# sabbirhossainujjal/LLMVoX

Hardware: AMD Instinct MI355X
Metric: speech tokens/sec (+ 24kHz audio samples/sec = 320 x tokens/s; p50 first-chunk latency) (higher is better)
Workload: dtype bf16

## Files before the change

llmvox_amd/csrc/ar_kernels.hip:

```cpp
#include "ar_plan.h"

#pragma clang fp contract(off)

namespace lvx {

#ifdef LVX_TIMING
constexpr int TS_BLOCKS = 1024;
__device__ uint64_t g_lvx_ts[16 * 4 * TS_BLOCKS * 4];
#define TS_DECL uint64_t ts_[2] = {0, 0}
#define TS_MARK(i) do { if (threadIdx.x == 0) ts_[i] = __builtin_amdgcn_s_memrealtime(); } while (0)
#define TS_SAVE(tag, layer, blk)                                                                    \
  do {                                                                                               \
    if (threadIdx.x == 0) {                                                                          \
      const uint64_t te_ = __builtin_amdgcn_s_memrealtime();                                         \
      const uint64_t hw_ = (uint64_t)__builtin_amdgcn_s_getreg((31 << 11) | 4) |                    \
                           ((uint64_t)__builtin_amdgcn_s_getreg((3 << 11) | 20) << 32);              \
      uint64_t* p_ = g_lvx_ts + ((size_t)(((tag) * 4 + (layer)) * TS_BLOCKS + min((int)(blk), TS_BLOCKS - 1))) * 4; \
      p_[0] = ts_[0]; p_[1] = ts_[1]; p_[2] = te_; p_[3] = hw_;                                      \
    }                                                                                                \
  } while (0)
#else
#define TS_DECL do {} while (0)
#define TS_MARK(i) do {} while (0)
#define TS_SAVE(tag, layer, blk) do {} while (0)
// ... 907 lines not shown
}
__device__ __forceinline__ void slot_update_bf16(float& m, float& l, f32x2_t (&o)[12], float sc, const uint4 (&vp)[3],
                                                 bool valid) {
  uint32_t v[12];
#pragma unroll
  for (int i = 0; i < 3; ++i) { v[4 * i] = vp[i].x; v[4 * i + 1] = vp[i].y; v[4 * i + 2] = vp[i].z; v[4 * i + 3] = vp[i].w; }
  if (!valid) return;
  const float mn = fmaxf(m, sc);
  const float alpha = __builtin_amdgcn_exp2f((m - mn) * 1.4426950408889634f);
  const float p = __builtin_amdgcn_exp2f((sc - mn) * 1.4426950408889634f);
  l = l * alpha + p;
  const f32x2_t a2 = f32x2_t{alpha, alpha}, p2 = f32x2_t{p, p};
#pragma unroll
  for (int j = 0; j < 12; ++j) {
    const f32x2_t vv = f32x2_t{__uint_as_float(v[j] << 16), __uint_as_float(v[j] & 0xffff0000u)};
    o[j] = __builtin_elementwise_fma(p2, vv, o[j] * a2);
  }
  m = mn;
}
__device__ __forceinline__ void slot_softmax_step_bf16(float& m, float& l, f32x2_t (&o)[12], const QSplit& qs,
                                                       const uint4 (&kp)[3], const uint4 (&vp)[3], bool valid) {
  slot_update_bf16(m, l, o, slot_score_bf16(qs, kp), vp, valid);
}

__device__ __forceinline__ float slot_fold_wave(float m, float& l, float (&o)[24]) {
  const float M = wave_max(m);
  const float f = (m == -INFINITY) ? 0.f : expf(m - M);
  l *= f;
#pragma unroll
  for (int i = 0; i < 24; ++i) o[i] *= f;
  return M;
}

template <typename TKV, int DEPTH, int NW, bool QKV = false>
__global__ __launch_bounds__(NW * 64) void ar_attn_v2_kernel(ArState st, int layer, int ns_max, int direct,
                                                         int selcopy) {
  constexpr int TK = NW * 16;
  constexpr bool SLOT = sizeof(TKV) < 4;
  static_assert(!QKV || (NW == 4 && sizeof(TKV) == 4), "the K-split c_attn: the fp32 parity mode's 4-wave blocks");
  constexpr int QH = QKV ? (3 * HD + NW * 64 - 1) / (NW * 64) : 1;
  __shared__ float wm_s[NW], wl_s[NW];
  __shared__ float wo_s[NW][4][HD];
  __shared__ float qs_s[QKV ? HD : 1];
  __shared__ __attribute__((aligned(16))) TKV kvh_s[QKV ? 2 : 1][QKV ? HD : 1];
  const int sp = blockIdx.x, head = blockIdx.y, b = blockIdx.z;
  const int tid = threadIdx.x, wave = tid >> 6, lane = tid & 63;
  TS_DECL;
  TS_MARK(0);
  const int4 ri = selcopy ? st.rowinfo_n[b] : st.rowinfo[b];
  float pq[QH][QKV ? 4 : 1];
  if constexpr (QKV) {
#pragma unroll
    for (int h = 0; h < QH; ++h) {
      const int e = min(tid + NW * 64 * h, 3 * HD - 1);
      const float* pp = st.qkvp + (size_t)b * (3 * D) + (e / HD) * D + head * HD + e % HD;
#pragma unroll
      for (int k = 0; k < 4; ++k) pq[h][k] = pp[(size_t)k * st.max_streams * (3 * D)];
    }
  }
  const bool cp = selcopy && sp == 0 && head == 0 && tid == 0;
  int jn = 0;
  if (cp) {
    jn = st.rowx_n[b].x;
    st.rowinfo[b] = ri;
    st.selrow[b] = 1u;
    if (b == 0) *st.selp = 0u;
  }
  auto copy_tail = [&]() {
    if (cp) st.rowx[b] = make_int2(jn, plan_tok(st, b, jn + 1));
  };
  const int s = ri.x;
  if (s < 0) {
    copy_tail();
    if (direct == ATTN_F32_ROWS && sp == 0 && tid < HD) st.part_o[(size_t)(b * N_HEAD + head) * NSPLIT * HD + tid] = 0.f;
    return;
  }
  const int t = ri.y + 1;
  const int ns = min(ns_max, (t + ATK - 1) / ATK);
  if (sp >= ns) return;
  const int chunk = SLOT ? (((t + ns - 1) / ns + ATK - 1) / ATK) * ATK : (t + ns - 1) / ns;
  const int k0 = sp * chunk, k1 = min(t, k0 + chunk);
  const size_t base = kv_at(layer, st.kv_chunks, st.max_streams, s, head, 0);
  const size_t cstride = (size_t)st.max_streams * N_HEAD * KV_CHUNK * HD;
  const TKV* __restrict__ Kg = reinterpret_cast<const TKV*>(st.kc) + base;
  const TKV* __restrict__ Vg = reinterpret_cast<const TKV*>(st.vc) + base;
  auto krow = [&](int k) { return (size_t)(k / KV_CHUNK) * cstride + (size_t)(k % KV_CHUNK) * HD; };
  const int part = tid & 3, kq = tid >> 2;
  float q[24];
  if constexpr (!QKV) {
    const float* qg = st.q + (size_t)b * D + head * HD + part * 24;
#pragma unroll
    for (int i = 0; i < 24; i += 4) {
      const float4 v = *reinterpret_cast<const float4*>(qg + i);
      q[i] = v.x * 0.10206207261596575f; q[i + 1] = v.y * 0.10206207261596575f;
      q[i + 2] = v.z * 0.10206207261596575f; q[i + 3] = v.w * 0.10206207261596575f;
    }
  }
  float m = -INFINITY, l = 0.f, o[24];
#pragma unroll
  for (int i = 0; i < 24; ++i) o[i] = 0.f;
  KvPiece<TKV> kpr[DEPTH][3], vpr[DEPTH][3];
  const int klast = ((k1 - 1) / ATK) * ATK;
  auto issue = [&](int kb, KvPiece<TKV>(&kp)[3], KvPiece<TKV>(&vp)[3]) {
    if constexpr (SLOT) {
      const size_t off = (size_t)min((kb / KV_CHUNK) + (kq / KV_CHUNK), klast / KV_CHUNK) * cstride +
                         (size_t)(kq % KV_CHUNK) * HD + part * 24;
#pragma unroll
      for (int i = 0; i < 3; ++i) {
        kp[i].load(Kg + off + i * 8);
        vp[i].load(Vg + off + i * 8);
      }
      return;
    }
    const int key = min(kb + kq, k1 - 1);
#pragma unroll
    for (int i = 0; i < 3; ++i) {
      kp[i].load(Kg + krow(key) + part * 24 + i * 8);
      vp[i].load(Vg + krow(key) + part * 24 + i * 8);
    }
  };
  constexpr bool BF = SLOT && sizeof(TKV) == 2;
  f32x2_t o2[BF ? 12 : 1];
// ... 44 lines not shown
    const float p = valid ? expf(sc - mn) : 0.f;
    l = l * alpha + wave_sum(part == 0 ? p : 0.f);
#pragma unroll
    for (int i = 0; i < 24; ++i) o[i] = fmaf(valid ? p : 0.f, valid ? vf[i] : 0.f, o[i] * alpha);
    m = mn;
  };
#pragma unroll
  for (int d = 0; d < DEPTH; ++d) issue(k0 + d * TK, kpr[d], vpr[d]);
  if constexpr (QKV) {
#pragma unroll
    for (int h = 0; h < QH; ++h) {
      const int e = tid + NW * 64 * h;
      float v = 0.f;
#pragma unroll
      for (int k = 0; k < 4; ++k) v += pq[h][k];
      if (e < HD) {
        qs_s[e] = v;
      } else if (e < 3 * HD && k1 == t) {
        const int which = e / HD - 1, d = e % HD;
        TKV hv;
        if constexpr (sizeof(TKV) == 4) hv = v;
        else if constexpr (sizeof(TKV) == 2) hv = f32_to_bf16(v);
        else hv = f32_to_fp8(v);
        kvh_s[which][d] = hv;
        reinterpret_cast<TKV*>(which ? st.vc : st.kc)[base + krow(ri.y) + d] = hv;
      }
    }
    asm volatile("s_waitcnt lgkmcnt(0)" ::: "memory");
    __builtin_amdgcn_s_barrier();
    asm volatile("" ::: "memory");
#pragma unroll
    for (int i = 0; i < 24; ++i) q[i] = qs_s[part * 24 + i] * 0.10206207261596575f;
  }
  if constexpr (BF) qsplit_make(q, qsp);
  for (int kb = k0; kb < k1; kb += DEPTH * TK) {
#pragma unroll
    for (int d = 0; d < DEPTH; ++d) {
      if (DEPTH == 2 && d > 0 && kb + d * TK >= k1) break;
      tile(kb + d * TK, kpr[d], vpr[d]);
      issue(kb + (d + DEPTH) * TK, kpr[d], vpr[d]);
      if (DEPTH > 2) __builtin_amdgcn_sched_barrier(0);
    }
  }
  if constexpr (BF) {
#pragma unroll
    for (int j = 0; j < 12; ++j) { o[2 * j] = o2[j].x; o[2 * j + 1] = o2[j].y; }
  }
  if constexpr (SLOT) {
    m = slot_fold_wave(m, l, o);
    l = wave_sum(part == 0 ? l : 0.f);
  }
#pragma unroll
  for (int i = 0; i < 24; ++i) {
    float v = o[i];
    v += dpp_f32<0x128>(v);
    v += dpp_f32<0x124>(v);
    o[i] = v;
  }
  if ((lane & 15) < 4) {
#pragma unroll
    for (int i = 0; i < 24; ++i) wo_s[wave][lane >> 4][(lane & 3) * 24 + i] = o[i];
  }
  TS_MARK(1);
  if (lane == 0) { wm_s[wave] = m; wl_s[wave] = l; }
  __syncthreads();
  TS_SAVE(2, layer, sp + gridDim.x * (head + N_HEAD * b));
  copy_tail();
  if (tid < HD) {
    float M = wm_s[0];
#pragma unroll
    for (int w = 1; w < NW; ++w) M = fmaxf(M, wm_s[w]);
    float ov = 0.f, lv = 0.f;
#pragma unroll
    for (int w = 0; w < NW; ++w) {
      const float f = (wm_s[w] == -INFINITY) ? 0.f : expf(wm_s[w] - M);
      ov += f * ((wo_s[w][0][tid] + wo_s[w][1][tid]) + (wo_s[w][2][tid] + wo_s[w][3][tid]));
      lv += f * wl_s[w];
    }
    if (direct == ATTN_F32_ROWS) {
      st.part_o[(size_t)(b * N_HEAD + head) * NSPLIT * HD + tid] = ov * (1.0f / lv);
      return;
    }
    if (direct) {
      st.xn[direct == ATTN_XN_PACKED ? xfrag(b, head * HD + tid, D) : (size_t)b * D + head * HD + tid] = f32_to_bf16(ov * (1.0f / lv));
      return;
    }
    st.part_o[((size_t)(b * N_HEAD + head) * NSPLIT + sp) * HD + tid] = ov;
    if (tid == 0) {
      float* ml = st.part_ml + ((size_t)(b * N_HEAD + head) * NSPLIT + sp) * 2;
      ml[0] = M;
      ml[1] = lv;
    }
  }
}

__device__ __forceinline__ void argmax_row(const ArState& st, int b, int4 ri, float* sv, float* sv2, int* si) {
  const int tid = threadIdx.x, wave = tid >> 6, lane = tid & 63;
  const float4* lg = reinterpret_cast<const float4*>(st.logits + (size_t)b * VOCAB);
  Best bt{-INFINITY, -INFINITY, 0x7fffffff};
#pragma unroll
  for (int j = 0; j < VOCAB / 1024; ++j) {
    const float4 v = lg[j * 256 + tid];
    const int i0 = (j * 256 + tid) * 4;
    bt = best_merge(bt, Best{v.x, -INFINITY, i0});
    bt = best_merge(bt, Best{v.y, -INFINITY, i0 + 1});
    bt = best_merge(bt, Best{v.z, -INFINITY, i0 + 2});
    bt = best_merge(bt, Best{v.w, -INFINITY, i0 + 3});
  }
  bt = best_wave(bt);
  if (lane == 0) { sv[wave] = bt.v; sv2[wave] = bt.v2; si[wave] = bt.i; }
  __syncthreads();
  if (wave == 0) {
    Best r{sv[0], sv2[0], si[0]};
    for (int w = 1; w < 4; ++w) r = best_merge(r, Best{sv[w], sv2[w], si[w]});
    r = softmax_ties(st.logits + (size_t)b * VOCAB, r, lane);
    if (lane == 0) argmax_commit(st, b, ri, r);
  }
}

__global__ __launch_bounds__(256) void ar_argmax_kernel(ArState st) {
  __shared__ float sv[4], sv2[4];
  __shared__ int si[4];
  const int b = blockIdx.x;
  const int4 ri = st.rowinfo[b];
  if (ri.x < 0) return;
  argmax_row(st, b, ri, sv, sv2, si);
// ... 181 lines not shown

__device__ __forceinline__ void embed_row(const GemvArgs& a, int4 ri, int lane, float4 (&v)[3], float* rden = nullptr) {
  if (ri.x < 0) {
#pragma unroll
    for (int j = 0; j < 3; ++j) v[j] = make_float4(0.f, 0.f, 0.f, 0.f);
    return;
  }
  const int p = ri.y, prev = ri.w;
  const int tok = ri.z < 0 ? 384 : ri.z;
  float4 pe[3];
  const float* wr_ = a.wpe + (size_t)p * D;
#pragma unroll
  for (int j = 0; j < 3; ++j) pe[j] = *reinterpret_cast<const float4*>(wr_ + j * 256 + lane * 4);
#pragma unroll
  for (int j = 0; j < 3; ++j) {
    const int k = j * 256 + lane * 4;
    v[j] = j == 0 ? *reinterpret_cast<const float4*>(a.text_table + (size_t)tok * TEXT_DIM + k)
                  : *reinterpret_cast<const float4*>(a.codebook + (size_t)prev * SPEECH_DIM + (k - TEXT_DIM));
  }
  if (ri.z < 0 && lane == 0) atomicOr(a.st.err, 2);
  float ss = 0.f;
#pragma unroll
  for (int j = 0; j < 3; ++j) {
    if (j > 0 && p == 0) v[j] = make_float4(0.f, 0.f, 0.f, 0.f);
    ss += (v[j].x * v[j].x + v[j].y * v[j].y) + (v[j].z * v[j].z + v[j].w * v[j].w);
  }
  const float den = fmaxf(sqrtf(wave_sum(ss)), 1e-8f);
  if (rden) *rden = 1.0f / den;
#pragma unroll
  for (int j = 0; j < 3; ++j)
    v[j] = make_float4(v[j].x / den + pe[j].x, v[j].y / den + pe[j].y, v[j].z / den + pe[j].z, v[j].w / den + pe[j].w);
}


template <int MODE>
__global__ __launch_bounds__(256) LVX_LOADS_FIRST void ar_rows_kernel(GemvArgs a) {
  const int tid = threadIdx.x, wave = tid >> 6, lane = tid & 63;
  const int b = blockIdx.x * (blockDim.x >> 6) + wave;
  if (b >= a.B) return;
  TS_DECL;
  TS_MARK(0);
  float4 g[3], v[3];
#pragma unroll
  for (int j = 0; j < 3; ++j) g[j] = *reinterpret_cast<const float4*>(a.ln_w + j * 256 + lane * 4);
  if (MODE == RMODE_LN || MODE == RMODE_LN_Y || MODE == RMODE_LN_Y_F32) {
    XRow<MODE == RMODE_LN_Y_F32 ? GIN_LN_Y : MODE> r;
    xrow_issue(a, b, lane, r);
    __builtin_amdgcn_sched_barrier(0);
    xrow_sum(r, v);
    if (MODE == RMODE_LN_Y || MODE == RMODE_LN_Y_F32)
#pragma unroll
      for (int j = 0; j < 3; ++j) *reinterpret_cast<float4*>(a.st.x + (size_t)b * D + j * 256 + lane * 4) = v[j];
  } else {
    const int4 ri = a.st.rowinfo[b];
    embed_row(a, ri, lane, v);
#pragma unroll
    for (int j = 0; j < 3; ++j) *reinterpret_cast<float4*>(a.st.x + (size_t)b * D + j * 256 + lane * 4) = v[j];
  }
  TS_MARK(1);
  wave_ln_regs(v, g);
  if constexpr (MODE == RMODE_LN_Y_F32 || MODE == RMODE_EMBED_F32) {
#pragma unroll
    for (int j = 0; j < 3; ++j) *reinterpret_cast<float4*>(a.st.h + (size_t)b * D + j * 256 + lane * 4) = v[j];
    return;
  }
  uint2* dst = reinterpret_cast<uint2*>(a.st.xn + (size_t)b * D);
#pragma unroll
  for (int j = 0; j < 3; ++j) {
    if (a.xpk) *reinterpret_cast<uint2*>(a.st.xn + xfrag(b, j * 256 + lane * 4, D)) = pack4_bf16(v[j]);
    else dst[j * 64 + lane] = pack4_bf16(v[j]);
  }
  TS_SAVE(a.N == VOCAB ? 8 : 0, a.layer, blockIdx.x);
}

template <bool F32OUT = false>
__global__ __launch_bounds__(256) LVX_LOADS_FIRST void ar_embed_select_kernel(GemvArgs a) {
  __shared__ float sv[4], sv2[4];
  __shared__ int si[4];
  const int b = blockIdx.x, tid = threadIdx.x, wave = tid >> 6, lane = tid & 63;
  TS_DECL;
  TS_MARK(0);
  int4 ri = a.st.rowinfo[b];
  const int2 rx = a.st.rowx[b];
  const unsigned pend = a.st.selrow[b];
  float4 g[3];
#pragma unroll
  for (int j = 0; j < 3; ++j) g[j] = *reinterpret_cast<const float4*>(a.ln_w + j * 256 + lane * 4);
  const float4* lg = reinterpret_cast<const float4*>(a.st.logits + (size_t)b * VOCAB);
  float4 lv[VOCAB / 1024];
#pragma unroll
  for (int k = 0; k < VOCAB / 1024; ++k) lv[k] = lg[k * 256 + tid];
  Best bt{-INFINITY, -INFINITY, 0x7fffffff};
#pragma unroll
  for (int k = 0; k < VOCAB / 1024; ++k) {
    const int i0 = (k * 256 + tid) * 4;
    bt = best_merge(bt, Best{lv[k].x, -INFINITY, i0});
    bt = best_merge(bt, Best{lv[k].y, -INFINITY, i0 + 1});
    bt = best_merge(bt, Best{lv[k].z, -INFINITY, i0 + 2});
    bt = best_merge(bt, Best{lv[k].w, -INFINITY, i0 + 3});
  }
  bt = best_wave(bt);
  TS_MARK(1);
  if (lane == 0) { sv[wave] = bt.v; sv2[wave] = bt.v2; si[wave] = bt.i; }
// ... 167 lines not shown
    bt = best_merge(bt, Best{lv[k].x, -INFINITY, i0});
    bt = best_merge(bt, Best{lv[k].y, -INFINITY, i0 + 1});
    bt = best_merge(bt, Best{lv[k].z, -INFINITY, i0 + 2});
    bt = best_merge(bt, Best{lv[k].w, -INFINITY, i0 + 3});
  }
  bt = best_wave(bt);
  if (lane == 0) { sv[wave] = bt.v; sv2[wave] = bt.v2; si[wave] = bt.i; }
  __syncthreads();
  int4 rn = ri;
  if (tk) {
    Best r{sv[0], sv2[0], si[0]};
#pragma unroll
    for (int w = 1; w < 4; ++w) r = best_merge(r, Best{sv[w], sv2[w], si[w]});
    r = softmax_ties(a.st.logits + (size_t)b * VOCAB, r, lane);
    const int sl = ri.x, p = ri.y + 1, j = rx.x;
    rn = make_int4(sl, min(p, a.st.max_pos - 1), rx.y, min(max(r.i, 0), VOCAB - 1));
    if (cx == 0 && tid == 0) {
      if (p >= a.st.max_pos) atomicOr(a.st.err, 1);
      if (j < a.st.plan_stride) {
        a.st.tok_plan[(size_t)b * a.st.plan_stride + j] = r.i;
        if (a.st.margin_plan) a.st.margin_plan[(size_t)b * a.st.plan_stride + j] = r.v - r.v2;
      }
      a.st.prev[sl] = r.i;
      a.st.pos[sl] = p;
      a.st.rowstep[b] = j + 1;
    }
  }
  if (cx == 0 && tid == 0) {
    a.st.rowinfo_n[b] = rn;
    a.st.rowx_n[b] = make_int2(tk ? rx.x + 1 : rx.x, 0);
  }
  const float tc = a.q0_code[(size_t)min(max(rn.w, 0), VOCAB - 1) * (3 * D) + n];
  if (wave == 0) {
    float4 v[3];
    float rden = 0.f;
    embed_row(a, rn, lane, v, &rden);
    if (cx == 0) {
#pragma unroll
      for (int j = 0; j < 3; ++j) *reinterpret_cast<float4*>(a.st.x + (size_t)b * D + j * 256 + lane * 4) = v[j];
    }
    float sm = 0.f;
#pragma unroll
    for (int j = 0; j < 3; ++j) sm += (v[j].x + v[j].y) + (v[j].z + v[j].w);
    const float mean = wave_sum(sm) * (1.0f / D);
    float qs = 0.f;
#pragma unroll
    for (int j = 0; j < 3; ++j) {
      const float4 d = make_float4(v[j].x - mean, v[j].y - mean, v[j].z - mean, v[j].w - mean);
      qs += (d.x * d.x + d.y * d.y) + (d.z * d.z + d.w * d.w);
    }
    const float rstd = 1.0f / sqrtf(wave_sum(qs) * (1.0f / D) + 1e-5f);
    if (lane == 0) sst = make_float4(rden, mean, rstd, 0.f);
  }
  __syncthreads();
  const float4 st = sst;
  const float cz = rn.y == 0 ? 0.f : 1.f;
  const float o = rn.x < 0 ? 0.f : st.z * (((tq + cz * tc) * st.x + tpo) - st.y * gq);
  if (n < D) {
    a.st.q[(size_t)b * D + n] = o;
  } else if (rn.x >= 0) {
    const int c = (n - D) % D, which = (n - D) / D;
    const int head = c / HD, d = c - head * HD;
    store_kv(a, which, kv_at(0, a.st.kv_chunks, a.st.max_streams, rn.x, head, rn.y) + d, o);
  }
  TS_SAVE(7, 0, cx + 9 * b);
}

template <int NS>
__global__ __launch_bounds__(256) void ar_merge_bf16_kernel(ArState st, int ns_max, int xpk) {
  __shared__ float cf[N_HEAD * NSPLIT];
  const int b = blockIdx.x, tid = threadIdx.x;
  const int4 ri = st.rowinfo[b];
  float2 ml = make_float2(-INFINITY, 0.f);
  if (tid < N_HEAD * NSPLIT) ml = reinterpret_cast<const float2*>(st.part_ml)[(size_t)b * N_HEAD * NSPLIT + tid];
  float pv[3][NS];
#pragma unroll
  for (int j = 0; j < 3; ++j) {
    const int e = tid + 256 * j, head = e / HD, d = e - head * HD;
    const float* po = st.part_o + ((size_t)(b * N_HEAD + head) * NSPLIT) * HD + d;
#pragma unroll
    for (int i = 0; i < NS; ++i) pv[j][i] = po[(size_t)i * HD];
  }
  if (tid < N_HEAD * NSPLIT) {
    const int ns = ri.x < 0 ? 0 : min(ns_max, (ri.y + 1 + 63) / 64);
    const bool on = (tid & (NSPLIT - 1)) < ns && ml.x != -INFINITY;
// ... 896 lines not shown
      break;
    case OP_LM_HEAD:
      a.W = w.w_lm; a.Wf = w.f_lm; a.N = VOCAB; a.ln_w = w.lnf;
      if (p.ksplit) {
        hipLaunchKernelGGL((ar_rows_kernel<RMODE_LN_Y_F32>), dim3(B), dim3(64), 0, s, a);
        launch_f32b<768, FIN_LN_ROWS, FOUT_LOGITS>(a, s);
      } else {
        launch_f32b<768, FIN_LN, FOUT_LOGITS>(a, s);
      }
      break;
  }
}

template <typename TW>
static bool launch_op(int op, GemvArgs& a, const ArWeights& w, int l, const ArStepPlan& p, hipStream_t s) {
  if (p.path == PATH_F32B || p.path == PATH_BT) {
    if (p.path == PATH_F32B) launch_op_f32b(op, a, w, l, p, s);
    else launch_op_bt(op, a, w, l, p, s);
    return true;
  }
  const int B = p.B;
  const bool ln = p.path == PATH_MFMA_LN, mf = ln || p.path == PATH_MFMA_ROWS, fm = p.fused_mlp;
  a.xpk = p.xpk;
  a.layer = l;
  a.yacc = mf ? a.st.yacc : nullptr;
  a.yfx = fm ? a.st.yfx : nullptr;
  a.add_y = l > 0;
  switch (op) {
    case OP_QKV:
      a.W = w.w_attn[l]; a.Wf = w.f_attn[l]; a.N = 3 * D; a.ln_w = w.ln1[l];
      if (!(p.sel == SEL_ARGMAX || (mf ? p.sel == SEL_EMBED || p.sel == SEL_Q0_ROWS || (ln && p.sel == SEL_LN_GRAN)
                                       : p.sel == SEL_GRAN)))
        ar_plan_bug(p, "c_attn");
      if (l == 0 && p.sel == SEL_LN_GRAN) {
        launch_mfma_ln<MLOUT_QKV, MLMODE_EMBED_SELECT>(a, s);
      } else if (l == 0 && p.sel == SEL_Q0_ROWS) {
        hipLaunchKernelGGL(ar_q0_rows_kernel, dim3(3 * D / 256, B), dim3(256), 0, s, a);
      } else if (l == 0 && p.sel == SEL_EMBED) {
        hipLaunchKernelGGL(ar_embed_select_kernel<>, dim3(B), dim3(256), 0, s, a);
        launch_mfma2<768, M2OUT_QKV>(a, s);
      } else if (ln) {
        if (l == 0) launch_mfma_ln<MLOUT_QKV, MLMODE_EMBED>(a, s);
        else launch_mfma_ln<MLOUT_QKV, MLMODE_LN_Y>(a, s);
      } else if (mf) {
        if (l == 0) hipLaunchKernelGGL((ar_rows_kernel<RMODE_EMBED>), dim3(B), dim3(64), 0, s, a);
        else hipLaunchKernelGGL((ar_rows_kernel<RMODE_LN_Y>), dim3(B), dim3(64), 0, s, a);
        launch_mfma2<768, M2OUT_QKV>(a, s);
      } else if (l == 0 && p.q0_gran) {
        hipLaunchKernelGGL(ar_q0_gran_kernel, dim3(3 * D / 256), dim3(256), 0, s, a);
      } else if (l == 0 && p.sel == SEL_GRAN) {
        launch_gemv<TW, 768, 1, 2, GIN_EMBED_SELECT, GOUT_QKV>(a, s);
      } else if (l == 0) {
        launch_gemv<TW, 768, 1, 2, GIN_EMBED, GOUT_QKV>(a, s);
      } else if (fm) {
        launch_gemv<TW, 768, 1, 2, GIN_LN_Y, GOUT_QKV>(a, s);
      } else {
        launch_gemv<TW, 768, 1, 2, GIN_LN, GOUT_QKV>(a, s);
      }
      break;
    case OP_ATTN:
      launch_attn(a.st, p.kv_dtype, B, l, s, p.nsplit, p.attn_direct, p.selcopy && l == 0, false, p.attn8);
      break;
    case OP_CPROJ:
      a.W = w.w_aproj[l]; a.Wf = w.f_aproj[l]; a.N = D;
      if (mf) {
        if (!ln) a.add_y = 0;
        if (p.nsplit > 1) launch_merge_bf16(a.st, B, p.nsplit, s, a.xpk);
        a.ln_w = w.ln2[l];
        if (!ln) launch_mfma2<768, M2OUT_RESID_STATS>(a, s, true);
        else launch_mfma2<768, M2OUT_RESID>(a, s);
      } else {
        launch_gemv<TW, 768, 1, 1, GIN_MERGE, GOUT_RESID>(a, s);
      }
      break;
    case OP_FC:
      a.W = w.w_fc[l]; a.Wf = w.f_fc[l]; a.N = DFF; a.ln_w = w.ln2[l];
      if (fm) {
        const bf16_t* wfc = reinterpret_cast<const bf16_t*>(w.w_fc[l]);
        const bf16_t* wpk = reinterpret_cast<const bf16_t*>(w.w_mproj_pk[l]);
        if (B <= 1) hipLaunchKernelGGL((ar_mlp_fused_kernel<1, 16>), dim3(DFF / 16), dim3(256), 0, s, a, wfc, wpk);
        else hipLaunchKernelGGL((ar_mlp_fused_kernel<2, 16>), dim3(DFF / 16), dim3(256), 0, s, a, wfc, wpk);
      } else if (ln) {
        launch_mfma_ln<MLOUT_GELU_BF16, MLMODE_LN>(a, s);
      } else if (mf) {
        a.gsum = w.fc_gsum[l];
        launch_mfma2<768, M2OUT_GELU_BF16, M2X_LN_AFTER>(a, s);
      } else {
        launch_gemv<TW, 768, 1, 2, GIN_LN, GOUT_GELU>(a, s);
      }
      break;
    case OP_MPROJ:
      a.W = w.w_mproj[l]; a.Wf = w.f_mproj[l]; a.N = D;
      if (fm) return false;
// ... 322 lines not shown
```

llmvox_amd/csrc/ar_plan.h:

```cpp
#pragma once
#include <stdio.h>
#include <stdlib.h>

#include "lvx_internal.h"

namespace lvx {

enum { OP_QKV = 0, OP_ATTN = 1, OP_CPROJ = 2, OP_FC = 3, OP_MPROJ = 4, OP_LM_HEAD = 5 };
enum { GIN_LN = 0, GIN_H = 1, GIN_MERGE = 2, GIN_EMBED = 3, GIN_LN_Y = 4, GIN_EMBED_SELECT = 5 };
enum { GOUT_QKV = 0, GOUT_RESID = 1, GOUT_GELU = 2, GOUT_LOGITS = 3, GOUT_SPLITK = 6, GOUT_LOGITS_GRAN = 9 };
enum { RMODE_LN = 0, RMODE_EMBED = 3, RMODE_LN_Y = 4, RMODE_LN_Y_F32 = 5, RMODE_EMBED_F32 = 6 };
enum { M2OUT_QKV = 0, M2OUT_RESID = 1, M2OUT_LOGITS = 3, M2OUT_GELU_BF16 = 5, M2OUT_SPLITK = 6, M2OUT_RESID_STATS = 7 };
enum { M2X_NONE = 0, M2X_LN_AFTER = 1 };
enum { MLOUT_QKV = 0, MLOUT_LOGITS = 3, MLOUT_GELU_BF16 = 5 };
enum { MLMODE_LN = 0, MLMODE_EMBED = 3, MLMODE_LN_Y = 4, MLMODE_EMBED_SELECT = 7 };
enum { BIN_LN = 0, BIN_ROWS = 1, BIN_EMBED = 3 };
enum { BOUT_QKV = 0, BOUT_RESID = 1, BOUT_LOGITS = 3, BOUT_GELU_BF16 = 5 };
enum { FIN_LN = 0, FIN_H = 1, FIN_MERGE = 2, FIN_EMBED = 3, FIN_ATTN_ROWS = 4, FIN_LN_ROWS = 6 };
enum { FOUT_QKV = 0, FOUT_RESID = 1, FOUT_GELU = 2, FOUT_LOGITS = 3, FOUT_SPLITK = 6 };
enum { ATTN_PARTIALS = 0, ATTN_XN = 1, ATTN_XN_PACKED = 2, ATTN_F32_ROWS = 3 };

enum ArPath { PATH_GEMV, PATH_MFMA_LN, PATH_MFMA_ROWS, PATH_BT, PATH_F32B };
enum ArSelect { SEL_ARGMAX = 0, SEL_GRAN = 1, SEL_EMBED = 2, SEL_LN_GRAN = 3, SEL_Q0_ROWS = 4, SEL_SAMPLE = 5 };
enum ArEndCommit { END_NONE, END_SELECT_FINAL, END_ARGMAX };

struct ArStepPlan {
  int B, kv_dtype;
  bool bf16, row;
  ArPath path;
  ArSelect sel;
  ArEndCommit end;
  int nsplit, attn_direct;
  bool attn8, selcopy;
  bool fused_mlp;
  bool q0_gran;
  int xpk;
  bool ksplit, qsplit;
};

constexpr int MFMA_BATCH_MIN = 3;
constexpr int LM8_ROWS = 8;
constexpr int ATTN_BLOCKS = 256;
inline int attn_ns_max(int B) {
  int ns = NSPLIT;
  while (ns > 1 && ns * N_HEAD * B > ATTN_BLOCKS) ns >>= 1;
  return ns;
}

[[noreturn]] inline void ar_plan_bug(const ArStepPlan& p, const char* where) {
  fprintf(stderr, "llmvox: %s: no kernel for select form %d on path %d at B = %d\n", where, (int)p.sel, (int)p.path, p.B);
  abort();
}

inline ArSelect ar_plan_select(const Opts& o, const ArStepPlan& p, bool q0) {
  if (!o.defer_select) return SEL_ARGMAX;
  if (p.path == PATH_GEMV) return p.B <= 2 ? SEL_GRAN : SEL_ARGMAX;
  if (p.B < 4) return SEL_ARGMAX;
  if (p.path == PATH_BT) return SEL_EMBED;
  if (p.path == PATH_F32B) return p.qsplit ? SEL_EMBED : SEL_ARGMAX;
  if (o.l0q && q0 && p.B <= 32) return SEL_Q0_ROWS;
  if (o.defer_select == 1 && p.path == PATH_MFMA_LN && p.B <= LM8_ROWS) return SEL_LN_GRAN;
  return SEL_EMBED;
}

inline ArStepPlan ar_plan_step(const Opts& o_, int wdtype, int kvdtype, int B, bool row, bool q0, bool sample = false) {
  sample = sample && !row;
  Opts o = o_;
  if (sample) o.defer_select = 0;
  ArStepPlan p{};
  p.B = B; p.kv_dtype = kvdtype; p.bf16 = wdtype == LVX_DTYPE_BF16; p.row = row;
  const bool batched = !row && B >= MFMA_BATCH_MIN && B <= 64;
  if (!batched || (!p.bf16 && !o.f32b)) p.path = PATH_GEMV;
  else if (!p.bf16) p.path = PATH_F32B;
  else if (o.bt && (B > 32 || o.bt == 2)) p.path = PATH_BT;
  else p.path = B <= o.ln_max ? PATH_MFMA_LN : PATH_MFMA_ROWS;
  const bool mf = p.path == PATH_MFMA_LN || p.path == PATH_MFMA_ROWS;
  p.ksplit = p.path == PATH_F32B && !(o.exp & 512);
  p.qsplit = p.ksplit && B <= 32 && !(o.exp & 1024);

  p.sel = row ? SEL_ARGMAX : sample ? SEL_SAMPLE : ar_plan_select(o, p, q0);
  p.end = p.sel == SEL_ARGMAX || p.sel == SEL_SAMPLE ? END_NONE : p.sel == SEL_GRAN ? END_SELECT_FINAL : END_ARGMAX;
  p.selcopy = p.sel == SEL_GRAN || p.sel == SEL_LN_GRAN || p.sel == SEL_Q0_ROWS;
  p.q0_gran = p.sel == SEL_GRAN && o.l0q && q0;
  p.fused_mlp = p.path == PATH_GEMV && p.bf16 && o.fuse_mlp && B <= 2;

  p.attn8 = mf && B >= 5 && (B <= 8 || (kvdtype == LVX_DTYPE_FP8 && B <= 16));
  p.nsplit = p.path == PATH_GEMV ? NSPLIT : (mf && (B > 8 || p.attn8)) ? 1 : attn_ns_max(B);
  p.xpk = (p.path == PATH_MFMA_ROWS && B <= 32) ? 1 : 0;
  p.attn_direct = p.nsplit > 1 || !(mf || p.path == PATH_F32B) ? ATTN_PARTIALS
                  : p.path == PATH_F32B ? ATTN_F32_ROWS : p.xpk ? ATTN_XN_PACKED : ATTN_XN;
  return p;
}

}
```

llmvox_amd/csrc/lvx_api.cpp:

```cpp
#include <hip/hip_runtime.h>

#include <cmath>
#include <cstdio>
#include <cstdlib>
#include <algorithm>
#include <atomic>
#include <cstring>
#include <functional>
#include <map>
#include <mutex>
#include <string>
#include <tuple>
#include <vector>

#include "llmvox.h"
#include "ar_plan.h"

using namespace lvx;

namespace lvx {
static const Opts kDefaultOpts{};
static thread_local const Opts* t_opts = nullptr;
const Opts& opts() { return t_opts ? *t_opts : kDefaultOpts; }
OptScope::OptScope(const Opts* o) : prev(t_opts) { t_opts = o; }
// ... 752 lines not shown
  return LVX_OK;
}

int lvx_stream_position(lvx_ctx* c, int slot, int* pos_out, void* stream) {
  NEED_FINAL(c);
  if (slot < 0 || slot >= c->cfg.max_streams || !pos_out) return fail(LVX_E_ARG, "bad slot/pos_out");
  HIP_TRY(hipSetDevice(c->cfg.device));
  int32_t v[2];
  launch_err_take(c->st.err, 1, 0, c->st.err + 3, (hipStream_t)stream);
  HIP_TRY(hipMemcpyAsync(&v[0], c->st.pos + slot, 4, hipMemcpyDeviceToHost, (hipStream_t)stream));
  HIP_TRY(hipMemcpyAsync(&v[1], c->st.err + 3, 4, hipMemcpyDeviceToHost, (hipStream_t)stream));
  HIP_TRY(hipStreamSynchronize((hipStream_t)stream));
  *pos_out = v[0];
  return bits_status(v[1]);
}

int lvx_set_option(lvx_ctx* c, const char* name, int value) {
  if (!c || !name) return fail(LVX_E_ARG, "null argument");
  std::string n(name);
  std::lock_guard<std::mutex> lk(c->mu);
  Opts& o = c->opts;
  if (n == "defer_select") o.defer_select = value;
  else if (n == "fuse_mlp") o.fuse_mlp = value != 0;
  else if (n == "bt") o.bt = std::min(std::max(value, 0), 2);
  else if (n == "codec_g2") o.codec_g2 = value != 0;
  else if (n == "codec_skinny") o.codec_skinny = value != 0;
  else if (n == "codec_g3") o.codec_g3 = value != 0;
  else if (n == "codec_g3f") o.codec_g3f = value == 1 ? 1 : 2;
  else if (n == "codec_exp") o.codec_exp = value;
  else if (n == "exp") o.exp = value;
  else if (n == "f32b") o.f32b = value != 0;
  else if (n == "ln_max") o.ln_max = std::min(std::max(value, 2), 8);
  else if (n == "l0q") o.l0q = value != 0;
  else return fail(LVX_E_NAME, "unknown option " + n);
  ++c->opt_epoch;
  return LVX_OK;
}

int lvx_set_capture_stream(lvx_ctx* c, void* stream) {
  if (!c) return fail(LVX_E_ARG, "null ctx");
  std::lock_guard<std::mutex> lk(c->mu);
  c->capture_stream = (hipStream_t)stream;
  return LVX_OK;
}

int lvx_set_graphs(lvx_ctx* c, int enable) {
  if (!c) return fail(LVX_E_ARG, "null ctx");
  c->use_graphs = enable != 0;
  return LVX_OK;
}

int lvx_ar_forward_row(lvx_ctx* c, int slot, int pos, const float* emb_row, float* logits, void* stream) {
  NEED_FINAL(c);
  if (slot < 0 || slot >= c->cfg.max_streams) return fail(LVX_E_ARG, "slot out of range");
  if (pos < 0 || pos >= BLOCK_SIZE)
    return fail(LVX_E_CAPACITY, "Cannot forward sequence of length " + std::to_string(pos + 1) +
                                    ", block size is only " + std::to_string(BLOCK_SIZE));
  if (pos >= c->cfg.max_positions)
    return fail(LVX_E_CAPACITY, "position " + std::to_string(pos) + " exceeds the KV capacity " +
                                    std::to_string(c->cfg.max_positions));
  if (!emb_row || !logits) return fail(LVX_E_ARG, "null emb_row/logits");
  HIP_TRY(hipSetDevice(c->cfg.device));
  const Opts o = c->opts_snapshot();
  OptScope os(&o);
  ar_launch_step(c->arw, c->st, ar_plan_step(o, c->cfg.weight_dtype, c->cfg.kv_dtype, 1, true, false), emb_row, slot,
                 pos, logits, (hipStream_t)stream);
// ... 693 lines not shown
```

llmvox_amd/csrc/lvx_internal.h:

```cpp
#pragma once
#include <hip/hip_runtime.h>
#include <stdint.h>
#include <string>

#include "lvx_common.h"
#include "llmvox.h"

namespace lvx {

constexpr int N_LAYER = 4, N_HEAD = 8, D = 768, HD = 96, DFF = 3072, VOCAB = 4096;
constexpr int TEXT_DIM = 256, SPEECH_DIM = 512, TEXT_VOCAB = 386, BLOCK_SIZE = 8192;
constexpr int NSPLIT = 16;
constexpr int KV_CHUNK = 64;
__host__ __device__ inline size_t kv_at(size_t layer, size_t chunks, size_t streams, int s, int head, int pos) {
  return (((((layer * chunks + (size_t)(pos / KV_CHUNK)) * streams + s) * 8 + head) * KV_CHUNK) + (size_t)(pos % KV_CHUNK)) * 96;
}
#ifndef LVX_YCOPIES
#define LVX_YCOPIES 4
#endif
constexpr int YCOPIES = LVX_YCOPIES;
constexpr int LM_MAX_BLOCKS = 1024;
struct Opts {
  int defer_select = 1;
  int fuse_mlp = 1;
  int bt = 1;
  int codec_g2 = 1, codec_skinny = 1, codec_g3 = 1, codec_g3f = 2;
  int codec_exp = 0;
  int exp = 0;
  int f32b = 1;
  int ln_max = 8;
  int l0q = 1;
};
const Opts& opts();
struct OptScope {
  explicit OptScope(const Opts* o);
  ~OptScope();
  OptScope(const OptScope&) = delete;
  OptScope& operator=(const OptScope&) = delete;
  const Opts* prev;
};

struct ArWeights {
  const float* wpe = nullptr;
  const float* text_table = nullptr;
  const float* codebook = nullptr;
  const float* ln1[N_LAYER] = {};
  const float* ln2[N_LAYER] = {};
  const float* lnf = nullptr;
  const void* w_attn[N_LAYER] = {};
  const void* w_aproj[N_LAYER] = {};
  const void* w_fc[N_LAYER] = {};
  const void* w_mproj[N_LAYER] = {};
  const void* w_mproj_pk[N_LAYER] = {};
  const float* fc_gsum[N_LAYER] = {};
  const void* w_lm = nullptr;
  const float* q0_text = nullptr;
  const float* q0_code = nullptr;
  const float* q0_pos = nullptr;
  const float* q0_g = nullptr;
  const void* f_attn[N_LAYER] = {};
  const void* f_aproj[N_LAYER] = {};
  const void* f_fc[N_LAYER] = {};
  const void* f_mproj[N_LAYER] = {};
  const void* f_lm = nullptr;
// ... 162 lines not shown
```

Baseline: 246,500.

## Fuse layer-0 argmax, embedding, QKV row build and attention into one kernel

Adds a fused layer-0 attention kernel that performs several steps inside each head block: the argmax/token selection from the previous logits, the embedding row statistics, the precomputed q0 QKV row synthesis and the new-token KV write, followed by attention over the cached tokens plus the new token. The separate q0_rows QKV launch is skipped, and the rowinfo/rowx copy moves into the layer-1 rows kernel. This removes kernel launches and global round trips in the small-batch decode step. In exchange, each head block redundantly reduces the full logit row, and the path is restricted to a single split with B>=9 and bf16/fp8 KV.

```diff
diff --git a/llmvox_amd/csrc/ar_kernels.hip b/llmvox_amd/csrc/ar_kernels.hip
--- a/llmvox_amd/csrc/ar_kernels.hip
+++ b/llmvox_amd/csrc/ar_kernels.hip
@@ -963,22 +963,81 @@
   return M;
 }
 
-template <typename TKV, int DEPTH, int NW, bool QKV = false>
-__global__ __launch_bounds__(NW * 64) void ar_attn_v2_kernel(ArState st, int layer, int ns_max, int direct,
-                                                         int selcopy) {
+__device__ __forceinline__ float4 q0_row_stats(const GemvArgs& a, int4 rn, int b, int lane, bool store_x);
+__device__ __forceinline__ int l0_next_tok(const ArState& st, int jn, int loaded) {
+  if (!st.text_plan) return 384;
+  return (jn + 1 < st.plan_stride) ? min(max(loaded, 0), TEXT_VOCAB - 1) : -1;
+}
+__device__ __forceinline__ void lds_barrier() {
+  asm volatile("s_waitcnt lgkmcnt(0)" ::: "memory");
+  __builtin_amdgcn_s_barrier();
+  asm volatile("" ::: "memory");
+}
+
+template <typename TKV, int DEPTH, int NW, bool QKV, bool L0>
+__device__ __forceinline__ void attn_v2_body(const ArState st, int layer, int ns_max, int direct, int selcopy,
+                                             const GemvArgs* a0) {
   constexpr int TK = NW * 16;
   constexpr bool SLOT = sizeof(TKV) < 4;
   static_assert(!QKV || (NW == 4 && sizeof(TKV) == 4), "the K-split c_attn: the fp32 parity mode's 4-wave blocks");
-  constexpr int QH = QKV ? (3 * HD + NW * 64 - 1) / (NW * 64) : 1;
+  static_assert(!L0 || (NW == 4 && SLOT && !QKV), "the fused layer-0 form: bf16 / fp8 KV in 4-wave blocks");
+  constexpr bool NEWKV = QKV || L0;
+  constexpr int QH = NEWKV ? (3 * HD + NW * 64 - 1) / (NW * 64) : 1;
   __shared__ float wm_s[NW], wl_s[NW];
   __shared__ float wo_s[NW][4][HD];
-  __shared__ float qs_s[QKV ? HD : 1];
-  __shared__ __attribute__((aligned(16))) TKV kvh_s[QKV ? 2 : 1][QKV ? HD : 1];
+  __shared__ float qs_s[NEWKV ? HD : 1];
+  __shared__ __attribute__((aligned(16))) TKV kvh_s[NEWKV ? 2 : 1][NEWKV ? HD : 1];
+  __shared__ float sv_s[L0 ? 4 : 1], sv2_s[L0 ? 4 : 1];
+  __shared__ int si_s[L0 ? 4 : 1];
+  __shared__ float4 sst_s;
   const int sp = blockIdx.x, head = blockIdx.y, b = blockIdx.z;
   const int tid = threadIdx.x, wave = tid >> 6, lane = tid & 63;
   TS_DECL;
   TS_MARK(0);
-  const int4 ri = selcopy ? st.rowinfo_n[b] : st.rowinfo[b];
+  int4 rold = make_int4(-1, 0, 0, 0);
+  int2 rx = make_int2(0, 0);
+  bool tk = false;
+  float4 lgv[L0 ? VOCAB / 1024 : 1];
+  int zn[L0 ? QH : 1];
+  float zg[L0 ? QH : 1], zt[L0 ? QH : 1], zp[L0 ? QH : 1];
+  int jnx = 0, tnext = 384;
+  int4 ri0 = make_int4(-1, 0, 0, 0);
+  if constexpr (L0) {
+    rold = st.rowinfo[b];
+    rx = st.rowx[b];
+    const unsigned pend = st.selrow[b];
+    const float4* lg = reinterpret_cast<const float4*>(st.logits + (size_t)b * VOCAB);
+#pragma unroll
+    for (int k = 0; k < VOCAB / 1024; ++k) lgv[k] = lg[k * 256 + tid];
+#pragma unroll
+    for (int h = 0; h < QH; ++h) {
+      const int e = min(tid + NW * 64 * h, 3 * HD - 1);
+      zn[h] = (e / HD) * D + head * HD + e % HD;
+      zg[h] = a0->q0_g[zn[h]];
+    }
+    tk = pend && rold.x >= 0;
+    const int p1 = min(max(tk ? rold.y + 1 : rold.y, 0), st.max_pos - 1);
+    const int t1 = tk ? rx.y : rold.z;
+#pragma unroll
+    for (int h = 0; h < QH; ++h) {
+      zt[h] = a0->q0_text[(size_t)(t1 < 0 ? 384 : t1) * (3 * D) + zn[h]];
+      zp[h] = a0->q0_pos[(size_t)p1 * (3 * D) + zn[h]];
+    }
+    jnx = tk ? rx.x + 1 : rx.x;
+    if (st.text_plan) tnext = st.text_plan[(size_t)b * st.plan_stride + min(jnx + 1, st.plan_stride - 1)];
+    ri0 = make_int4(rold.x, p1, 0, 0);
+    if (rold.x < 0) {
+      if (head == 0) {
+        if (tid == 0) {
+          st.rowinfo_n[b] = rold;
+          st.rowx_n[b] = make_int2(jnx, l0_next_tok(st, jnx, tnext));
+        }
+        if (tid < D / 4) reinterpret_cast<float4*>(st.x + (size_t)b * D)[tid] = make_float4(0.f, 0.f, 0.f, 0.f);
+      }
+      return;
+    }
+  }
+  const int4 ri = L0 ? ri0 : selcopy ? st.rowinfo_n[b] : st.rowinfo[b];
   float pq[QH][QKV ? 4 : 1];
   if constexpr (QKV) {
 #pragma unroll
@@ -1010,7 +1069,7 @@
   const int ns = min(ns_max, (t + ATK - 1) / ATK);
   if (sp >= ns) return;
   const int chunk = SLOT ? (((t + ns - 1) / ns + ATK - 1) / ATK) * ATK : (t + ns - 1) / ns;
-  const int k0 = sp * chunk, k1 = min(t, k0 + chunk);
+  const int k0 = sp * chunk, k1 = L0 ? t - 1 : min(t, k0 + chunk);
   const size_t base = kv_at(layer, st.kv_chunks, st.max_streams, s, head, 0);
   const size_t cstride = (size_t)st.max_streams * N_HEAD * KV_CHUNK * HD;
   const TKV* __restrict__ Kg = reinterpret_cast<const TKV*>(st.kc) + base;
@@ -1018,7 +1077,7 @@
   auto krow = [&](int k) { return (size_t)(k / KV_CHUNK) * cstride + (size_t)(k % KV_CHUNK) * HD; };
   const int part = tid & 3, kq = tid >> 2;
   float q[24];
-  if constexpr (!QKV) {
+  if constexpr (!NEWKV) {
     const float* qg = st.q + (size_t)b * D + head * HD + part * 24;
 #pragma unroll
     for (int i = 0; i < 24; i += 4) {
@@ -1129,6 +1188,73 @@
 #pragma unroll
     for (int i = 0; i < 24; ++i) q[i] = qs_s[part * 24 + i] * 0.10206207261596575f;
   }
+  if constexpr (L0) {
+    const GemvArgs& a = *a0;
+    Best bt{-INFINITY, -INFINITY, 0x7fffffff};
+#pragma unroll
+    for (int k = 0; k < VOCAB / 1024; ++k) {
+      const int i0 = (k * 256 + tid) * 4;
+      bt = best_merge(bt, Best{lgv[k].x, -INFINITY, i0});
+      bt = best_merge(bt, Best{lgv[k].y, -INFINITY, i0 + 1});
+      bt = best_merge(bt, Best{lgv[k].z, -INFINITY, i0 + 2});
+      bt = best_merge(bt, Best{lgv[k].w, -INFINITY, i0 + 3});
+    }
+    bt = best_wave(bt);
+    if (lane == 0) { sv_s[wave] = bt.v; sv2_s[wave] = bt.v2; si_s[wave] = bt.i; }
+    lds_barrier();
+    int4 rn = rold;
+    if (tk) {
+      Best r{sv_s[0], sv2_s[0], si_s[0]};
+#pragma unroll
+      for (int w = 1; w < 4; ++w) r = best_merge(r, Best{sv_s[w], sv2_s[w], si_s[w]});
+      r = softmax_ties(st.logits + (size_t)b * VOCAB, r, lane);
+      const int sl = rold.x, p = rold.y + 1, j = rx.x;
+      rn = make_int4(sl, min(p, st.max_pos - 1), rx.y, min(max(r.i, 0), VOCAB - 1));
+      if (head == 0 && tid == 0) {
+        if (p >= st.max_pos) atomicOr(st.err, 1);
+        if (j < st.plan_stride) {
+          st.tok_plan[(size_t)b * st.plan_stride + j] = r.i;
+          if (st.margin_plan) st.margin_plan[(size_t)b * st.plan_stride + j] = r.v - r.v2;
+        }
+        st.prev[sl] = r.i;
+        st.pos[sl] = p;
+        st.rowstep[b] = j + 1;
+      }
+    }
+    if (head == 0 && tid == 0) {
+      st.rowinfo_n[b] = rn;
+      st.rowx_n[b] = make_int2(jnx, l0_next_tok(st, jnx, tnext));
+    }
+    float zc[QH];
+#pragma unroll
+    for (int h = 0; h < QH; ++h) zc[h] = a.q0_code[(size_t)min(max(rn.w, 0), VOCAB - 1) * (3 * D) + zn[h]];
+    if (wave == 0) {
+      const float4 s4 = q0_row_stats(a, rn, b, lane, head == 0);
+      if (lane == 0) sst_s = s4;
+    }
+    lds_barrier();
+    const float4 ss = sst_s;
+    const float cz = rn.y == 0 ? 0.f : 1.f;
+#pragma unroll
+    for (int h = 0; h < QH; ++h) {
+      const int e = tid + NW * 64 * h;
+      const float v = ss.z * (((zt[h] + cz * zc[h]) * ss.x + zp[h]) - ss.y * zg[h]);
+      if (e < HD) {
+        qs_s[e] = v;
+      } else if (e < 3 * HD) {
+        const int which = e / HD - 1, d = e % HD;
+        TKV hv;
+        if constexpr (sizeof(TKV) == 2) hv = f32_to_bf16(v);
+        else hv = f32_to_fp8(v);
+        kvh_s[which][d] = hv;
+        reinterpret_cast<TKV*>(which ? st.vc : st.kc)[base + krow(ri.y) + d] = hv;
+      }
+    }
+    lds_barrier();
+#pragma unroll
+    for (int i = 0; i < 24; ++i) q[i] = qs_s[part * 24 + i] * 0.10206207261596575f;
+    TS_MARK(1);
+  }
   if constexpr (BF) qsplit_make(q, qsp);
   for (int kb = k0; kb < k1; kb += DEPTH * TK) {
 #pragma unroll
@@ -1138,6 +1264,27 @@
       issue(kb + (d + DEPTH) * TK, kpr[d], vpr[d]);
       if (DEPTH > 2) __builtin_amdgcn_sched_barrier(0);
     }
+  }
+  if constexpr (L0) {
+    const bool mine = kq == (t - 1) % TK;
+    KvPiece<TKV> kx[3], vx[3];
+#pragma unroll
+    for (int i = 0; i < 3; ++i) {
+      kx[i].load(kvh_s[0] + part * 24 + i * 8);
+      vx[i].load(kvh_s[1] + part * 24 + i * 8);
+    }
+    if constexpr (BF) {
+      uint4 ku[3], vu[3];
+#pragma unroll
+      for (int i = 0; i < 3; ++i) { ku[i] = reinterpret_cast<const uint4&>(kx[i]); vu[i] = reinterpret_cast<const uint4&>(vx[i]); }
+      slot_softmax_step_bf16(m, l, o2, qsp, ku, vu, mine);
+    } else {
+      float kf[24], vf[24];
+#pragma unroll
+      for (int i = 0; i < 3; ++i) { kx[i].get(kf + 8 * i); vx[i].get(vf + 8 * i); }
+      slot_softmax_step(m, l, o, q, kf, vf, mine);
+    }
+    TS_SAVE(9, layer, head + N_HEAD * b);
   }
   if constexpr (BF) {
 #pragma unroll
@@ -1189,6 +1336,17 @@
       ml[1] = lv;
     }
   }
+}
+
+template <typename TKV, int DEPTH, int NW, bool QKV = false>
+__global__ __launch_bounds__(NW * 64) void ar_attn_v2_kernel(ArState st, int layer, int ns_max, int direct,
+                                                         int selcopy) {
+  attn_v2_body<TKV, DEPTH, NW, QKV, false>(st, layer, ns_max, direct, selcopy, nullptr);
+}
+
+template <typename TKV>
+__global__ __launch_bounds__(256) LVX_LOADS_FIRST void ar_attn_l0_kernel(GemvArgs a, int direct) {
+  attn_v2_body<TKV, 2, 4, false, true>(a.st, 0, 1, direct, 0, &a);
 }
 
 __device__ __forceinline__ void argmax_row(const ArState& st, int b, int4 ri, float* sv, float* sv2, int* si) {
@@ -1436,9 +1594,33 @@
     v[j] = make_float4(v[j].x / den + pe[j].x, v[j].y / den + pe[j].y, v[j].z / den + pe[j].z, v[j].w / den + pe[j].w);
 }
 
-
-template <int MODE>
+__device__ __forceinline__ float4 q0_row_stats(const GemvArgs& a, int4 rn, int b, int lane, bool store_x) {
+  float4 v[3];
+  float rden = 0.f;
+  embed_row(a, rn, lane, v, &rden);
+  if (store_x) {
+#pragma unroll
+    for (int j = 0; j < 3; ++j) *reinterpret_cast<float4*>(a.st.x + (size_t)b * D + j * 256 + lane * 4) = v[j];
+  }
+  float sm = 0.f;
+#pragma unroll
+  for (int j = 0; j < 3; ++j) sm += (v[j].x + v[j].y) + (v[j].z + v[j].w);
+  const float mean = wave_sum(sm) * (1.0f / D);
+  float qs = 0.f;
+#pragma unroll
+  for (int j = 0; j < 3; ++j) {
+    const float4 d = make_float4(v[j].x - mean, v[j].y - mean, v[j].z - mean, v[j].w - mean);
+    qs += (d.x * d.x + d.y * d.y) + (d.z * d.z + d.w * d.w);
+  }
+  const float rstd = 1.0f / sqrtf(wave_sum(qs) * (1.0f / D) + 1e-5f);
+  return make_float4(rden, mean, rstd, 0.f);
+}
+
+
+template <int MODE_>
 __global__ __launch_bounds__(256) LVX_LOADS_FIRST void ar_rows_kernel(GemvArgs a) {
+  constexpr bool COPY = MODE_ == RMODE_LN_Y_COPY;
+  constexpr int MODE = COPY ? RMODE_LN_Y : MODE_;
   const int tid = threadIdx.x, wave = tid >> 6, lane = tid & 63;
   const int b = blockIdx.x * (blockDim.x >> 6) + wave;
   if (b >= a.B) return;
@@ -1447,9 +1629,15 @@
   float4 g[3], v[3];
 #pragma unroll
   for (int j = 0; j < 3; ++j) g[j] = *reinterpret_cast<const float4*>(a.ln_w + j * 256 + lane * 4);
+  int4 rcp = make_int4(0, 0, 0, 0);
+  int2 rxcp = make_int2(0, 0);
   if (MODE == RMODE_LN || MODE == RMODE_LN_Y || MODE == RMODE_LN_Y_F32) {
     XRow<MODE == RMODE_LN_Y_F32 ? GIN_LN_Y : MODE> r;
     xrow_issue(a, b, lane, r);
+    if constexpr (COPY) {
+      rcp = a.st.rowinfo_n[b];
+      rxcp = a.st.rowx_n[b];
+    }
     __builtin_amdgcn_sched_barrier(0);
     xrow_sum(r, v);
     if (MODE == RMODE_LN_Y || MODE == RMODE_LN_Y_F32)
@@ -1473,6 +1661,14 @@
   for (int j = 0; j < 3; ++j) {
     if (a.xpk) *reinterpret_cast<uint2*>(a.st.xn + xfrag(b, j * 256 + lane * 4, D)) = pack4_bf16(v[j]);
     else dst[j * 64 + lane] = pack4_bf16(v[j]);
+  }
+  if constexpr (COPY) {
+    if (lane == 0) {
+      a.st.rowinfo[b] = rcp;
+      a.st.rowx[b] = rxcp;
+      a.st.selrow[b] = 1u;
+      if (b == 0) *a.st.selp = 0u;
+    }
   }
   TS_SAVE(a.N == VOCAB ? 8 : 0, a.layer, blockIdx.x);
 }
@@ -1706,25 +1902,8 @@
   }
   const float tc = a.q0_code[(size_t)min(max(rn.w, 0), VOCAB - 1) * (3 * D) + n];
   if (wave == 0) {
-    float4 v[3];
-    float rden = 0.f;
-    embed_row(a, rn, lane, v, &rden);
-    if (cx == 0) {
-#pragma unroll
-      for (int j = 0; j < 3; ++j) *reinterpret_cast<float4*>(a.st.x + (size_t)b * D + j * 256 + lane * 4) = v[j];
-    }
-    float sm = 0.f;
-#pragma unroll
-    for (int j = 0; j < 3; ++j) sm += (v[j].x + v[j].y) + (v[j].z + v[j].w);
-    const float mean = wave_sum(sm) * (1.0f / D);
-    float qs = 0.f;
-#pragma unroll
-    for (int j = 0; j < 3; ++j) {
-      const float4 d = make_float4(v[j].x - mean, v[j].y - mean, v[j].z - mean, v[j].w - mean);
-      qs += (d.x * d.x + d.y * d.y) + (d.z * d.z + d.w * d.w);
-    }
-    const float rstd = 1.0f / sqrtf(wave_sum(qs) * (1.0f / D) + 1e-5f);
-    if (lane == 0) sst = make_float4(rden, mean, rstd, 0.f);
+    const float4 s4 = q0_row_stats(a, rn, b, lane, cx == 0);
+    if (lane == 0) sst = s4;
   }
   __syncthreads();
   const float4 st = sst;
@@ -2687,7 +2866,8 @@
       if (!(p.sel == SEL_ARGMAX || (mf ? p.sel == SEL_EMBED || p.sel == SEL_Q0_ROWS || (ln && p.sel == SEL_LN_GRAN)
                                        : p.sel == SEL_GRAN)))
         ar_plan_bug(p, "c_attn");
-      if (l == 0 && p.sel == SEL_LN_GRAN) {
+      if (l == 0 && p.l0_fused) {
+      } else if (l == 0 && p.sel == SEL_LN_GRAN) {
         launch_mfma_ln<MLOUT_QKV, MLMODE_EMBED_SELECT>(a, s);
       } else if (l == 0 && p.sel == SEL_Q0_ROWS) {
         hipLaunchKernelGGL(ar_q0_rows_kernel, dim3(3 * D / 256, B), dim3(256), 0, s, a);
@@ -2699,6 +2879,7 @@
         else launch_mfma_ln<MLOUT_QKV, MLMODE_LN_Y>(a, s);
       } else if (mf) {
         if (l == 0) hipLaunchKernelGGL((ar_rows_kernel<RMODE_EMBED>), dim3(B), dim3(64), 0, s, a);
+        else if (l == 1 && p.l0_fused) hipLaunchKernelGGL((ar_rows_kernel<RMODE_LN_Y_COPY>), dim3(B), dim3(64), 0, s, a);
         else hipLaunchKernelGGL((ar_rows_kernel<RMODE_LN_Y>), dim3(B), dim3(64), 0, s, a);
         launch_mfma2<768, M2OUT_QKV>(a, s);
       } else if (l == 0 && p.q0_gran) {
@@ -2714,6 +2895,14 @@
       }
       break;
     case OP_ATTN:
+      if (l == 0 && p.l0_fused) {
+        if (p.kv_dtype == LVX_DTYPE_BF16)
+          hipLaunchKernelGGL(ar_attn_l0_kernel<bf16_t>, dim3(1, N_HEAD, B), dim3(256), 0, s, a, p.attn_direct);
+        else if (p.kv_dtype == LVX_DTYPE_FP8)
+          hipLaunchKernelGGL(ar_attn_l0_kernel<fp8_t>, dim3(1, N_HEAD, B), dim3(256), 0, s, a, p.attn_direct);
+        else ar_plan_bug(p, "fused layer-0 attention");
+        break;
+      }
       launch_attn(a.st, p.kv_dtype, B, l, s, p.nsplit, p.attn_direct, p.selcopy && l == 0, false, p.attn8);
       break;
     case OP_CPROJ:
diff --git a/llmvox_amd/csrc/ar_plan.h b/llmvox_amd/csrc/ar_plan.h
--- a/llmvox_amd/csrc/ar_plan.h
+++ b/llmvox_amd/csrc/ar_plan.h
@@ -9,7 +9,7 @@
 enum { OP_QKV = 0, OP_ATTN = 1, OP_CPROJ = 2, OP_FC = 3, OP_MPROJ = 4, OP_LM_HEAD = 5 };
 enum { GIN_LN = 0, GIN_H = 1, GIN_MERGE = 2, GIN_EMBED = 3, GIN_LN_Y = 4, GIN_EMBED_SELECT = 5 };
 enum { GOUT_QKV = 0, GOUT_RESID = 1, GOUT_GELU = 2, GOUT_LOGITS = 3, GOUT_SPLITK = 6, GOUT_LOGITS_GRAN = 9 };
-enum { RMODE_LN = 0, RMODE_EMBED = 3, RMODE_LN_Y = 4, RMODE_LN_Y_F32 = 5, RMODE_EMBED_F32 = 6 };
+enum { RMODE_LN = 0, RMODE_EMBED = 3, RMODE_LN_Y = 4, RMODE_LN_Y_F32 = 5, RMODE_EMBED_F32 = 6, RMODE_LN_Y_COPY = 7 };
 enum { M2OUT_QKV = 0, M2OUT_RESID = 1, M2OUT_LOGITS = 3, M2OUT_GELU_BF16 = 5, M2OUT_SPLITK = 6, M2OUT_RESID_STATS = 7 };
 enum { M2X_NONE = 0, M2X_LN_AFTER = 1 };
 enum { MLOUT_QKV = 0, MLOUT_LOGITS = 3, MLOUT_GELU_BF16 = 5 };
@@ -32,6 +32,7 @@
   ArEndCommit end;
   int nsplit, attn_direct;
   bool attn8, selcopy;
+  bool l0_fused;
   bool fused_mlp;
   bool q0_gran;
   int xpk;
@@ -86,6 +87,7 @@
 
   p.attn8 = mf && B >= 5 && (B <= 8 || (kvdtype == LVX_DTYPE_FP8 && B <= 16));
   p.nsplit = p.path == PATH_GEMV ? NSPLIT : (mf && (B > 8 || p.attn8)) ? 1 : attn_ns_max(B);
+  p.l0_fused = o.l0a && p.sel == SEL_Q0_ROWS && p.nsplit == 1 && !p.attn8 && B >= 9 && kvdtype != LVX_DTYPE_F32;
   p.xpk = (p.path == PATH_MFMA_ROWS && B <= 32) ? 1 : 0;
   p.attn_direct = p.nsplit > 1 || !(mf || p.path == PATH_F32B) ? ATTN_PARTIALS
                   : p.path == PATH_F32B ? ATTN_F32_ROWS : p.xpk ? ATTN_XN_PACKED : ATTN_XN;
diff --git a/llmvox_amd/csrc/lvx_api.cpp b/llmvox_amd/csrc/lvx_api.cpp
--- a/llmvox_amd/csrc/lvx_api.cpp
+++ b/llmvox_amd/csrc/lvx_api.cpp
@@ -808,6 +808,7 @@
   else if (n == "f32b") o.f32b = value != 0;
   else if (n == "ln_max") o.ln_max = std::min(std::max(value, 2), 8);
   else if (n == "l0q") o.l0q = value != 0;
+  else if (n == "l0a") o.l0a = value != 0;
   else return fail(LVX_E_NAME, "unknown option " + n);
   ++c->opt_epoch;
   return LVX_OK;
diff --git a/llmvox_amd/csrc/lvx_internal.h b/llmvox_amd/csrc/lvx_internal.h
--- a/llmvox_amd/csrc/lvx_internal.h
+++ b/llmvox_amd/csrc/lvx_internal.h
@@ -30,6 +30,7 @@
   int f32b = 1;
   int ln_max = 8;
   int l0q = 1;
+  int l0a = 1;
 };
 const Opts& opts();
 struct OptScope {
```

Result: faster. 249,800, median of 6 (+1.3%).
